# gooofy/zerovox

Hardware: AMD Instinct MI355X
Metric: audio samples/sec + RTF, 128-phoneme zero-shot synth @22.05kHz, 1/2/4/8 GPU (higher is better)
Workload: dtype f16+bf16

## Files before the change

### zerovox_amd/build.py

```python
import os
import subprocess
import sys

HERE = os.path.dirname(os.path.abspath(__file__))
CSRC = os.path.join(HERE, "csrc")
LIB = os.path.join(HERE, "libzvx.so")
KTEST_SRC = os.path.join(os.path.dirname(HERE), "tests", "native", "zvx_ktest.hip")
KTEST_LIB = os.path.join(HERE, "libzvx_ktest.so")
SOURCES = ["gemm.hip", "resstream.hip", "pairstream.hip", "narrowstage.hip", "attention.hip", "ops.hip", "spectral.hip", "zvx.hip"]
UNITS = [("gemm", "gemm.hip", ["-DZVX_GEMM_PART=1"]), ("gemm_resfuse", "gemm.hip", ["-DZVX_GEMM_PART=2"])] + \
        [(s_[:-4], s_, []) for s_ in SOURCES[1:]]
FLAGS = ["--offload-arch=gfx950", "-O3", "-std=c++17", "-fPIC", "-Wall", "-Wno-unused-function", "-Wno-inline-asm"]
EXTRA_FLAGS = {"gemm.hip": ["-fno-honor-nans"], "pairstream.hip": ["-fno-honor-nans"], "narrowstage.hip": ["-fno-honor-nans"], "resstream.hip": ["-fno-honor-nans"] + (["-DRS_PROFILE"] if os.environ.get("ZVX_RS_PROFILE_BUILD") else [])}


def _stale(target, deps):
    if not os.path.exists(target):
        return True
    t = os.path.getmtime(target)
    return any(os.path.getmtime(d) > t for d in deps)


def _parse_resources(text):
    import re
    res, cur = {}, None
    keys = {"TotalSGPRs": "sgprs", "VGPRs": "vgprs", "AGPRs": "agprs", "ScratchSize [bytes/lane]": "scratch", "Occupancy [waves/SIMD]": "occupancy",
            "SGPRs Spill": "sgpr_spill", "VGPRs Spill": "vgpr_spill", "LDS Size [bytes/block]": "lds"}
    for line in text.splitlines():
        m = re.search(r"remark:\s+Function Name: (\S+)", line)
        if m:
            cur = res.setdefault(m.group(1), {})
            continue
        m = re.search(r"remark:\s+([A-Za-z \[\]/]+): (\d+)", line)
        if m and cur is not None and m.group(1).strip() in keys:
            cur[keys[m.group(1).strip()]] = int(m.group(2))
    return res


def resources():
    import json
    out = {}
    for stem, _src, _defs in UNITS:
        f = os.path.join(CSRC, stem + ".resources.json")
        if os.path.exists(f):
            out.update(json.load(open(f)))
    return out


def build(force: bool = False, verbose: bool = True) -> str:
    hipcc = os.environ.get("HIPCC", "/opt/rocm/bin/hipcc")
    headers = [os.path.join(CSRC, "zvx_kernels.h"), os.path.join(CSRC, "mfma_util.h"), os.path.join(os.path.dirname(HERE), "include", "zvx.h")]
    def compile_one(unit):
        stem, src, defs = unit
        s = os.path.join(CSRC, src)
        o = os.path.join(CSRC, stem + ".o")
        rj = os.path.join(CSRC, stem + ".resources.json")
        if force or _stale(o, [s] + headers) or not os.path.exists(rj):
            cmd = [hipcc] + FLAGS + EXTRA_FLAGS.get(src, []) + defs + ["-Rpass-analysis=kernel-resource-usage", "-c", s, "-o", o]
            if verbose:
                print(" ".join(cmd), flush=True)
            p = subprocess.run(cmd, stderr=subprocess.PIPE, text=True)
            lines, keep, skip = p.stderr.splitlines(), [], 0
            for l in lines:
                if "[-Rpass-analysis=kernel-resource-usage]" in l:
                    skip = 2
                elif skip and (l.lstrip().startswith("|") or (l.strip()[:1].isdigit() and " | " in l)):
# ... 43 lines not shown
```

### zerovox_amd/csrc/gemm.hip

```cpp
#include "mfma_util.h"
#include "zvx_kernels.h"

#include <cstring>
#include <type_traits>

#ifndef ZVX_GEMM_PART
#define ZVX_GEMM_PART 0
#endif
#define ZVX_PART_MAIN (ZVX_GEMM_PART != 2)
#define ZVX_PART_RESFUSE (ZVX_GEMM_PART != 1)
#if ZVX_GEMM_PART == 2
extern thread_local bool zvx_gemm_dry_run;
#else
thread_local hipEvent_t zvx_gemm_ev_start = nullptr, zvx_gemm_ev_stop = nullptr;
thread_local bool zvx_gemm_dry_run = false;
#endif
#define g_dry_run zvx_gemm_dry_run

#define ZVX_LAUNCH(...) do { if (!g_dry_run) ZVX_DISPATCH(__VA_ARGS__); } while (0)

namespace zvx {


#define PITCH 80
// ... 774 lines not shown
    uint4 w[NT][KS];
    {
        const uint4* Wq = (const uint4*)a.Wp + ((long)wc * NT * 4) * 64 + lane;
#pragma unroll
        for (int t = 0; t < NT; t++)
#pragma unroll
            for (int kk = 0; kk < KS; kk++) w[t][kk] = Wq[(t * 4 + kk) * 64];
    }
    {
        const bool flat = MAXH > 64 && a.flat_win;
        const int in_rows = flat ? a.flat_rows : in_len;
#pragma unroll
        for (int h0 = 0; h0 < NIT; h0 += FCH) {
            uint4 sv[FCH];
#pragma unroll
            for (int i = 0; i < FCH; i++) {
                const int c = tid + (h0 + i) * 256;
                const int row = c / CPR, q = c % CPR;
                const int g = m0 - HL + row;
                sv[i] = make_uint4(0, 0, 0, 0);
                if (h0 + i < NIT && c < SR * CPR && g >= 0 && g < in_rows && (!flat || (g % a.flat_win) < in_len)) sv[i] = *(const uint4*)(Xp + (long)g * a.ldx + q * 8);
            }
#pragma unroll
            for (int i = 0; i < FCH; i++) {
                const int c = tid + (h0 + i) * 256;
                if (h0 + i < NIT && c < SR * CPR) *(uint4*)(slab + (c / CPR) * PITCH_ + (c % CPR) * 16) = sv[i];
            }
        }
    }
    __syncthreads();

    f32x16 acc[1][TM];
#pragma unroll
    for (int j = 0; j < TM; j++)
#pragma unroll
        for (int e = 0; e < 16; e++) acc[0][j][e] = 0.f;
    const int xrow0 = HL + wr * (BM / WM) + (lane & 31);
    const int koff = (lane >> 5) * 16;
#pragma unroll
    for (int t = 0; t < NT; t++) {
        const unsigned char* rowp = slab + (xrow0 + a.dv[t]) * PITCH_ + koff;
#pragma unroll
        for (int kk = 0; kk < KS; kk++)
#pragma unroll
            for (int j = 0; j < TM; j++) {
                const uint4 xf = *(const uint4*)(rowp + j * 32 * PITCH_ + kk * 32);
                acc[0][j] = mfma16<F16>(w[t][kk], xf, acc[0][j]);
            }
    }
    __syncthreads();
    epilogue_rows<TM, 1>(a, acc, b, m0 + wr * (BM / WM), wc * 32, out_len, lane, slab + wave * (32 * (32 * 4 + 16)));
}

typedef __attribute__((ext_vector_type(2))) unsigned u32x2_t;
__device__ __forceinline__ void store_block_mfma_layout(unsigned short* row_ptr , const uint2 (&pk)[4], int lane, bool ok) {
#pragma unroll
    for (int pr = 0; pr < 2; pr++) {
        const u32x2_t sx = __builtin_amdgcn_permlane32_swap(pk[2 * pr].x, pk[2 * pr + 1].x, false, false);
        const u32x2_t sy = __builtin_amdgcn_permlane32_swap(pk[2 * pr].y, pk[2 * pr + 1].y, false, false);
        if (ok) *(u32x4*)(row_ptr + 8 * (2 * pr + (lane >> 5))) = (u32x4){sx.x, sy.x, sx.y, sy.y};
    }
}

template <int C, int BM, int WM, int WN, int MAXH, int MODE, int WGPC, bool POOL = false>
__global__ __launch_bounds__(WM * WN * 64, WM * WN * WGPC / 4) void conv2d_persist_kernel(const GemmArgs a, const int ntm, const int ntiles) {
    constexpr int NTHR = WM * WN * 64;
    constexpr int NT = 9, TM = BM / WM / 32, KS = C / 16, PITCH_ = C * 2 + 16, CPR = C / 8, RSTEP = NTHR / CPR;
    constexpr int NIT = ((BM + MAXH) * CPR + NTHR - 1) / NTHR;
    constexpr bool EC_LDS = NTHR > 256;
    static_assert(WN * 32 == C && BM % (WM * 32) == 0, "wave layout");
    extern __shared__ __attribute__((aligned(16))) unsigned char slab[];

    const int tid = threadIdx.x, lane = tid & 63, wave = __builtin_amdgcn_readfirstlane(tid >> 6);
    const int wr = wave % WM, wc = wave / WM;
    const int G = gridDim.x, xcd = blockIdx.x & 7, slot = blockIdx.x >> 3;
    auto tile_of = [&](int r) {
        const int base = r * G, n = ntiles - base < G ? ntiles - base : G;
        if (n <= 0) return ntiles;
        const int per = (n + 7) >> 3, t = xcd * per + slot;
        return (slot < per && t < n) ? base + t : ntiles;
    };
    const int HL = a.halo_l, SR = BM + a.halo_l + a.halo_r, win = a.flat_win, in_rows = a.flat_rows;

    uint4 w[NT][KS];
    {
        const uint4* Wq = (const uint4*)a.Wp + ((long)wc * NT * 4) * 64 + lane;
#pragma unroll
        for (int t = 0; t < NT; t++)
#pragma unroll
            for (int kk = 0; kk < KS; kk++) w[t][kk] = Wq[(t * 4 + kk) * 64];
    }
    float* const ecl = (float*)(slab + ((SR * PITCH_ + 15) & ~15));
    float4 ec0[EC_LDS ? 1 : 4], ec1[(MODE == 1 && !EC_LDS) ? 4 : 1];
    if (EC_LDS) {
        if (tid < C) { ecl[tid] = MODE == 0 ? a.bias[tid] : a.post_scale[tid]; if (MODE == 1) ecl[C + tid] = a.post_shift[tid]; }
    } else {
#pragma unroll
        for (int g = 0; g < 4; g++) {
            const int ch = wc * 32 + 8 * g + 4 * (lane >> 5);
            if (MODE == 0) ec0[g] = *(const float4*)(a.bias + ch);
            else { ec0[g] = *(const float4*)(a.post_scale + ch); ec1[g] = *(const float4*)(a.post_shift + ch); }
        }
    }
    u32x4 sv[NIT];
    const int row_t = tid / CPR, q8 = (tid % CPR) * 8;
    auto request = [&](int t) __attribute__((always_inline)) {
        const int b = t / ntm, m0 = (t - b * ntm) * BM;
        const int in_len = a.in_len[b];
        const __amdgpu_buffer_rsrc_t rs = __builtin_amdgcn_make_buffer_rsrc((void*)((const unsigned short*)a.X + (long)b * a.x_bs), 0, in_rows * a.ldx * 2, 0x00020000);
        int g = m0 - HL + row_t;
        int col = (g + 2 * win) % win;
#pragma unroll
        for (int it = 0; it < NIT; it++) {
            const bool ok = tid + it * NTHR < SR * CPR && g >= 0 && g < in_rows && col < in_len;
            sv[it] = __builtin_amdgcn_raw_buffer_load_b128(rs, ok ? (g * a.ldx + q8) * 2 : (int)0x80000000, 0, 0);
// ... 761 lines not shown
        if (a.ntaps == 3) { ZVX_RFP_MODE(3) }
        if (a.ntaps == 7) { ZVX_RFP_MODE(7) }
        if constexpr (C <= 32) { if (a.ntaps == 11) { ZVX_RFP_MODE(11) } }
    }
#undef ZVX_RFP_MODE
#undef ZVX_RFP
    return false;
}

int launch_resfuse(GemmArgs a, hipStream_t stream) {
    if (a.dtype == DT_F32 || !a.Wp || !a.Wp2 || a.N != a.K || a.nheads != 1 || a.wout > 0) return -1;
    if (!(a.ntaps == 3 || a.ntaps == 7 || a.ntaps == 11)) return -1;
    int h1 = 0;
    for (int i = 0; i < a.ntaps; i++) { const int d = a.dv1[i] < 0 ? -a.dv1[i] : a.dv1[i]; if (d > h1) h1 = d; }
    if (h1 > 32) return -1;
    a.halo_l = a.halo_r = h1;
    a.fused = 1;
    if (a.N == 128 && a.no_pairstream != 1) {
        const int h2 = (a.ntaps - 1) / 2, dil = a.dv1[1] - a.dv1[0];
        bool ok = a.alpha == 1.f && a.bias_mode == 1 && !a.post_scale && (!a.out || a.out_dtype == a.dtype) && a.res_mode == 2 && a.res_dtype == a.dtype &&
                  a.res == a.X && a.r_bs == a.x_bs && a.ldr == a.ldx && (!a.accum || a.accum_dtype == a.dtype) && (a.act == ACT_NONE || a.act == ACT_LRELU) &&
                  (a.accum_mode || a.out_scale == 1.f) && a.in_len == a.out_len;
        for (int t = 0; t < a.ntaps; t++) ok = ok && a.dv[t] == t - h2 && a.dv1[t] == (t - h2) * dil;
        if (ok) {
            PairArgs p;
            memset(&p, 0, sizeof p);
            p.X = a.X; p.x_bs = a.x_bs; p.ldx = a.ldx; p.W1 = a.Wp2; p.W2 = a.Wp; p.b1 = a.bias1; p.b2 = a.bias;
            p.C = a.N; p.ntaps = a.ntaps; p.dil = dil;
            p.out = a.out; p.o_bs = a.o_bs; p.ldo = a.ldo;
            p.accum = a.accum; p.a_bs = a.a_bs; p.lda = a.lda; p.accum_mode = a.accum ? a.accum_mode : 0;
            p.slope1 = a.slope1; p.res_inv_slope = a.res_inv_slope; p.out_scale = a.out_scale; p.slope = a.act == ACT_LRELU ? a.slope : 1.f;
            p.f16 = a.dtype == DT_F16;
            p.len = a.out_len; p.M = a.M; p.nbatch = a.nbatch; p.force = a.no_pairstream == 2;
            if (launch_pairstream(p, stream, g_dry_run)) return 23;
        }
    }
    {
        if (a.N == 32 && launch_resfuse_persist_c<32>(a, stream)) return 16;
        if (a.N == 64 && a.ntaps != 11 && launch_resfuse_persist_c<64>(a, stream)) return 17;
        if (a.N == 64 && a.ntaps == 11 && launch_resfuse_persist_c<64, 1>(a, stream)) return 17;
    }
    return -1;
}
#endif
#if ZVX_PART_MAIN

struct Variant { const char* name; int dt, bm, bn; };
static const Variant kVariants[] = {
    {"gemm_bf16_128x128", DT_BF16, 128, 128}, {"gemm_bf16_256x64", DT_BF16, 256, 64},
    {"gemm_bf16_256x32", DT_BF16, 256, 32},   {"gemm_f32_128x128", DT_F32, 128, 128},
    {"gemm_f32_256x64", DT_F32, 256, 64},     {"gemm_f32_256x32", DT_F32, 256, 32},
    {"convslab_bf16_128x256", DT_BF16, 128, 256}, {"convslab_bf16_256x128", DT_BF16, 256, 128},
    {"convslab_bf16_256x64", DT_BF16, 256, 64},   {"convslab_bf16_256x32", DT_BF16, 256, 32},
    {"(unused)", DT_BF16, 0, 0}, {"resfuse_bf16_c8", DT_BF16, 256, 8}, {"resfuse_bf16_c16", DT_BF16, 256, 16}, {"resfuse_bf16_c128", DT_BF16, 64, 128},
    {"convreg_bf16_c32", DT_BF16, 512, 32},       {"convreg_bf16_c64", DT_BF16, 256, 64},
    {"resfuse_bf16_c32", DT_BF16, 256, 32},       {"resfuse_bf16_c64", DT_BF16, 128, 64},
    {"gemm_bf16_64x64", DT_BF16, 64, 64},         {"gemm_f32_64x64", DT_F32, 64, 64},
    {"resstream_bf16_c32", DT_BF16, 64, 32},      {"resstream_bf16_c64", DT_BF16, 32, 64},
    {"convslab_bf16_128x128", DT_BF16, 128, 128},
    {"pairstream_bf16_c128", DT_BF16, 128, 128},
    {"narrowstage_c16", DT_BF16, 256, 16}, {"narrowstage_c8", DT_BF16, 512, 8},
    {"conv2d_persist_c32", DT_BF16, 384, 32}, {"conv2d_persist_c64", DT_BF16, 256, 64},
    {"conv2d_s2_c32", DT_BF16, 256, 64}, {"conv2d_s2_c64", DT_BF16, 128, 128},
    {"rb2fuse_bf16_c32", DT_BF16, 256, 32}, {"rb2fuse_bf16_c64", DT_BF16, 256, 64},
};
const char* gemm_variant_name(int id) { return kVariants[id].name; }
int gemm_num_variants() { return (int)(sizeof(kVariants) / sizeof(kVariants[0])); }


template <int BM, int BN, int WM, int WN, int MINW, int R, int EPI = -1>
static void launch_slab_variant(const GemmArgs& a, dim3 grid, size_t lds, hipStream_t stream) {
    const bool fullk = a.K % SLAB_KC == 0 && a.K2 == 0;
    if constexpr (R == 0 || EPI == -1 || EPI == ZVX_EPI(0, 0, 1) || EPI == ZVX_EPI_FLIP) {
        if (a.dtype == DT_F16) {
            if (fullk) ZVX_LAUNCH((convslab_kernel<BM, BN, WM, WN, true, MINW, R, EPI, 64, true>), grid, dim3(256), lds, stream, a);
            else if constexpr (EPI != ZVX_EPI_FLIP) ZVX_LAUNCH((convslab_kernel<BM, BN, WM, WN, false, MINW, R, EPI, 64, true>), grid, dim3(256), lds, stream, a);
            return;
        }
    }
    if constexpr (EPI < 0 || !(EPI & 16)) {
        if (fullk) ZVX_LAUNCH((convslab_kernel<BM, BN, WM, WN, true, MINW, R, EPI>), grid, dim3(256), lds, stream, a);
        else if constexpr (EPI != ZVX_EPI_FLIP) ZVX_LAUNCH((convslab_kernel<BM, BN, WM, WN, false, MINW, R, EPI>), grid, dim3(256), lds, stream, a);
    }
}

int gemm_epi_mode_of(const GemmArgs& a) {
    if (a.alpha == 1.f && !a.post_scale && a.out && a.out_dtype != a.dtype && a.dtype != DT_F32 && a.out_dtype != DT_F32 && !a.out_split3 && a.bias_mode == 1 && a.bias &&
        (a.act == ACT_NONE || a.act == ACT_LRELU) && !a.res_mode && !(a.accum && a.accum_mode) && a.out_scale == 1.f && a.K % SLAB_KC == 0 && !a.K2) return ZVX_EPI_FLIP;
    if (a.alpha != 1.f || a.post_scale || (a.out && a.out_dtype != a.dtype) || a.dtype == DT_F32 || a.out_split3 || a.bias_mode == 2) return -1;
    const int am = a.accum ? a.accum_mode : 0;
    if (a.dtype == DT_F16 && a.out && !am && a.act == ACT_NONE && a.res_mode <= 1 && (!a.res_mode || a.res_dtype == DT_F16) && (a.res_mode || a.out_scale != 1.f) &&
        (a.bias_mode == 0 || a.bias)) return ZVX_EPI_DEC(a.res_mode ? 1 : 0);
    if (a.bias_mode != 1 || !a.bias) return -1;
    if (a.act != ACT_NONE && a.act != ACT_LRELU) return -1;
    if (a.res_mode && (a.res_mode != 2 || a.res_dtype != a.dtype)) return -1;
    if (am && a.accum_dtype != a.dtype) return -1;
    if (!am && a.out_scale != 1.f) return -1;
    if (!a.out && !(am & 2)) return -1;
    const int e = ZVX_EPI(a.res_mode ? 1 : 0, am, a.out ? 1 : 0);
    switch (e) {
        case ZVX_EPI(0, 0, 1): case ZVX_EPI(1, 0, 1): case ZVX_EPI(1, 2, 0): case ZVX_EPI(1, 3, 0): case ZVX_EPI(1, 1, 1): return e;
    }
    return -1;
}

static int launch_convslab(GemmArgs a, hipStream_t stream) {
    const bool bflat_hint = a.bflat != 0;
// ... 247 lines not shown
```

### zerovox_amd/csrc/mfma_util.h

```cpp
#pragma once
#include <hip/hip_runtime.h>

namespace zvx {

typedef __attribute__((ext_vector_type(8))) __bf16 bf16x8;
typedef __attribute__((ext_vector_type(16))) float f32x16;
typedef __attribute__((ext_vector_type(4))) float f32x4;
typedef __attribute__((ext_vector_type(4))) unsigned int u32x4;
typedef __attribute__((ext_vector_type(4))) int i32x4;
typedef float f32x2 __attribute__((ext_vector_type(2)));

__device__ __forceinline__ unsigned pack_bf16x2(float lo, float hi) {
    typedef __attribute__((ext_vector_type(2))) __bf16 bf16x2_t;
    bf16x2_t v = {(__bf16)lo, (__bf16)hi};
    return __builtin_bit_cast(unsigned, v);
}
__device__ __forceinline__ f32x2 unpack_bf16x2(unsigned u) { return (f32x2){__uint_as_float(u << 16), __uint_as_float(u & 0xffff0000u)}; }
__device__ __forceinline__ f32x2 lrelu2(f32x2 v, float slope) { const f32x2 m = v * slope; return (f32x2){fmaxf(v.x, m.x), fmaxf(v.y, m.y)}; }
__device__ __forceinline__ f32x2 inv_lrelu2(f32x2 y, float inv_slope) { const f32x2 m = y * inv_slope; return (f32x2){fminf(y.x, m.x), fminf(y.y, m.y)}; }

typedef __attribute__((ext_vector_type(8))) _Float16 f16x8;
typedef _Float16 f16x2_t __attribute__((ext_vector_type(2)));
__device__ __forceinline__ void f16_saturate_mode() { asm volatile("s_setreg_imm32_b32 hwreg(HW_REG_MODE, 23, 1), 1"); }
__device__ __forceinline__ unsigned pack_f16x2_raw(float lo, float hi) { const f16x2_t v = {(_Float16)lo, (_Float16)hi}; return __builtin_bit_cast(unsigned, v); }
__device__ __forceinline__ unsigned pack_f16x2_sat(float lo, float hi) { return pack_f16x2_raw(__builtin_amdgcn_fmed3f(lo, -65504.f, 65504.f), __builtin_amdgcn_fmed3f(hi, -65504.f, 65504.f)); }
__device__ __forceinline__ f32x2 unpack_f16x2(unsigned u) { const f16x2_t v = __builtin_bit_cast(f16x2_t, u); return (f32x2){(float)v.x, (float)v.y}; }
template <bool H> __device__ __forceinline__ unsigned pack16(float lo, float hi) { if constexpr (H) return pack_f16x2_raw(lo, hi); else return pack_bf16x2(lo, hi); }
template <bool H> __device__ __forceinline__ f32x2 unpack16(unsigned u) { if constexpr (H) return unpack_f16x2(u); else return unpack_bf16x2(u); }
template <bool H> __device__ __forceinline__ f32x16 mfma16(const uint4& a, const uint4& b, const f32x16& c) {
    if constexpr (H) return __builtin_amdgcn_mfma_f32_32x32x16_f16(__builtin_bit_cast(f16x8, a), __builtin_bit_cast(f16x8, b), c, 0, 0, 0);
    else return __builtin_amdgcn_mfma_f32_32x32x16_bf16(__builtin_bit_cast(bf16x8, a), __builtin_bit_cast(bf16x8, b), c, 0, 0, 0);
}
template <bool H> __device__ __forceinline__ f32x16 mfma16(const u32x4& a, const uint4& b, const f32x16& c) { return mfma16<H>(__builtin_bit_cast(uint4, a), b, c); }

}
```

### zerovox_amd/csrc/zvx.hip

```cpp
#include "../../include/zvx.h"
#include "zvx_kernels.h"

#include <dlfcn.h>
#include <math.h>
#include <cmath>
#include <rccl/rccl.h>
#include <stdarg.h>
#include <stdio.h>
#include <string.h>

#include <algorithm>
#include <map>
#include <sstream>
#include <stdexcept>
#include <string>
#include <vector>

using namespace zvx;

namespace {

struct ZvxError : std::runtime_error {
    int code;
    ZvxError(int c, const std::string& m) : std::runtime_error(m), code(c) {}
// ... 47 lines not shown
    hipEvent_t ev_aux[2] = {nullptr, nullptr};
    int va_overlap_maxb = 1 << 20;
    ncclComm_t comm = nullptr;
    int rank = 0, world = 1;
    hipEvent_t ev_compute = nullptr;
    std::map<const void*, hipEvent_t> gather_fence;
    std::string err;
    std::map<std::string, std::string> cfg;
    std::map<std::string, Tensor> tensors;
    std::vector<float> host_blob;
    std::map<std::string, DevBuf> bufs;
    std::map<const void*, const void*> packed;
    std::map<const void*, const void*> pair_packed;
    int dt = DT_BF16;
    int H = 0, emb_dim = 0, punct_dim = 0, n_phone_rows = 0, n_punct_rows = 0, max_txt_len = 0, max_mel_len = 0;
    int enc_layers = 0, enc_heads = 0, ffn_dim = 0, ffn_k0 = 0, ffn_k1 = 0, vp_dim = 0, vp_k = 0, n_bins = 0;
    int dec_layers = 0, dec_heads = 0, dec_scln = 0, n_mels = 0, hop = 0, res_dim = 0, dec_kind = 0, rn_asp = 1;
    std::vector<int> rn_layers, rn_filters, voc_rates, voc_ksizes, voc_rb_k;
    std::vector<std::vector<int>> voc_rb_d;
    int voc_resblock = 1, voc_c0 = 0;
    int B = 0, Tmax = 0, Lmax = 0;
    std::vector<int> T_host, mel_len_host;
    std::vector<int> in_stage;
    bool have_features = false, have_mel = false;
    int profile = 0;
    int profile_only = -1;
    int rs_prof = 0;
    int enc_split = 0;
    const void* fft_xs_ready = nullptr;
    int norm_fuse_maxb = 1 << 20;
    int dec_sc_fuse = 1;
    int dec_flat = 1;
    int voc_f16_stages = -1;
    int voc_h16_ok = -1;
    int voc_f16 = 1;
    int dec_f16 = 1;
    int use_attn_f32 = 1;
    int use_flash = 1;
    int use_resstream = 1;
    int rs_seg_min = 0;
    int spk_s2_fuse = 1;
    int spk_pool_fuse = 1;
    int slab_small = 2, slab_flat = 1;
    int poison_pads = 0;
    int sat_check = 0;
    unsigned long long* sat_count_dev() { return (unsigned long long*)buf("sat.count", 64); }
    void sat_scan(const void* x, int dt, long bs, int ld, int B, int rows_max, const int* rows, int C) {
        if (sat_check && x && dt == DT_F16) launch_count_sat16(x, bs, ld, B, rows_max, rows, C, sat_count_dev(), stream);
    }
    int use_rb2fuse = 1;
    int use_stagefuse = 1;
    struct NsWeights { void* W = nullptr; float* bias = nullptr; int woff[18] = {0}; };
    std::map<std::string, NsWeights> ns_weights;
    int use_pairstream = 1;
    int shape_log = 0;
    int max_frames = 1 << 18;
    int out_rate = 0;
    struct RsBank { int L = 0, M = 0, half = 0, T = 0, pitch = 0; const float* dev = nullptr; };
    std::map<std::pair<int, int>, RsBank> rs_banks;
    std::map<int, const double*> lim_wins;
    std::map<int, LoudCoef> loud_coefs;
    struct DnTables { int n_fft = 0, log2n = 0, win_length = 0; const float* twid = nullptr; const float* win = nullptr; const double* win2 = nullptr; double den_min = 0; };
    DnTables dn_tab;
    void* join_host = nullptr;
    size_t join_host_cap = 0;
    void* join_pinned(size_t bytes) {
        if (bytes > join_host_cap) {
            if (join_host) { HIPCHK(hipStreamSynchronize(stream)); HIPCHK(hipHostFree(join_host)); join_host = nullptr; join_host_cap = 0; }
            const size_t cap = bytes + bytes / 8 + 256;
            HIPCHK(hipHostMalloc(&join_host, cap, hipHostMallocDefault));
            join_host_cap = cap;
        }
        return join_host;
    }
    hipEvent_t stage_ev[ZVX_T_COUNT][2];
    bool stage_used[ZVX_T_COUNT];
    float stage_ms[ZVX_T_COUNT];
    std::vector<GemmEvent> pending;
    std::vector<zvx_kernel_stat> stats;
    std::string tag = "other";
    std::map<std::string, zvx_kernel_stat> tagstats;
    std::map<std::string, zvx_kernel_stat> namedstats;
    std::vector<hipEvent_t> event_pool;

    int cfg_int(const char* k) const {
        auto it = cfg.find(k);
        if (it == cfg.end()) fail(ZVX_E_MANIFEST, "manifest: missing cfg '%s'", k);
        return atoi(it->second.c_str());
    }
    std::vector<int> cfg_list(const char* k) const {
        auto it = cfg.find(k);
        if (it == cfg.end()) fail(ZVX_E_MANIFEST, "manifest: missing cfg '%s'", k);
        std::vector<int> v; std::stringstream ss(it->second); std::string tok;
        while (std::getline(ss, tok, ',')) if (!tok.empty()) v.push_back(atoi(tok.c_str()));
        return v;
    }
    const Tensor& t(const std::string& name) const {
        auto it = tensors.find(name);
        if (it == tensors.end()) fail(ZVX_E_MANIFEST, "weights: tensor '%s' missing", name.c_str());
        return it->second;
    }
    bool has(const std::string& name) const { return tensors.count(name) != 0; }
    const float* pf(const std::string& name) const { return (const float*)t(name).dev; }

    void drain_for_free() {
        HIPCHK(hipStreamSynchronize(stream));
// ... 1010 lines not shown
struct VocStage {
    int i, Cin, Cout, rows_in, rows;
    const int* len_in; const int* len;
    int dt_in, dt;
    float next_slope;
};

struct RbConv { std::string name; const Tensor* w = nullptr; const void* packed = nullptr; const float* bias = nullptr; };
struct RbWeights { std::string name; std::vector<RbConv> c1, c2; };
RbWeights voc_rb_weights(zvx_ctx* c, const VocCall& v, const VocStage& s, int j) {
    RbWeights w;
    w.name = "voc.rb" + std::to_string(s.i * v.nk + j);
    auto conv = [&](const char* which, int t) {
        RbConv r;
        r.name = w.name + which + std::to_string(t);
        r.w = &voc_weight(c, r.name + "_w", s.dt);
        auto it = c->packed.find(r.w->dev);
        if (it != c->packed.end()) r.packed = it->second;
        r.bias = c->pf(r.name + "_b");
        return r;
    };
    for (int t = 0; t < (int)c->voc_rb_d[j].size(); t++) {
        if (c->voc_resblock == 1) { w.c1.push_back(conv(".c1_", t)); w.c2.push_back(conv(".c2_", t)); }
        else w.c1.push_back(conv(".c_", t));
    }
    return w;
}

struct StageClose { int accum_mode; bool writes_out; };
StageClose stage_close(int j, int nk) {
    if (nk == 1) return {0, true};
    return {j == 0 ? 2 : (j < nk - 1 ? 3 : 1), j == nk - 1};
}
template <typename Args>
void close_stage(Args& a, const StageClose& cl, const VocCall& v, const VocStage& s) {
    a.accum = cl.accum_mode ? v.XS : nullptr; a.accum_mode = cl.accum_mode; a.a_bs = (long)s.rows * s.Cout; a.lda = s.Cout;
    if (cl.writes_out) { a.out = v.A; a.out_scale = 1.0f / v.nk; a.slope = s.next_slope; }
    else a.out = nullptr;
    if constexpr (std::is_same<Args, GemmArgs>::value) { a.accum_dtype = s.dt; if (cl.writes_out) a.act = ACT_LRELU; }
}

void voc_conv_pre(zvx_ctx* c, const VocCall& v, const void* vin, int dt) {
    const int nm = c->n_mels, Pmax = v.Pmax;
    const int* P_d = v.lens_d + v.B;
    GemmArgs a = gemm_base(dt);
    a.X = vin; a.x_bs = (long)Pmax * nm; a.ldx = nm; a.W = voc_weight(c, "voc.pre_w", dt).dev; a.ldw = nm; a.w_ts = (long)c->voc_c0 * nm;
    a.M = Pmax; a.N = c->voc_c0; a.K = nm; a.nbatch = v.B; a.in_len = P_d; a.out_len = P_d;
    set_taps_1d(a, c->t("voc.pre_w").dim(0), 1);
    a.bias = c->pf("voc.pre_b"); a.bias_mode = 1; a.act = ACT_LRELU; a.slope = 0.1f;
    a.out = v.A; a.o_bs = (long)Pmax * c->voc_c0; a.ldo = c->voc_c0;
    c->gemm(a);
}

void voc_upsample(zvx_ctx* c, const VocCall& v, const VocStage& s) {
    const int u = c->voc_rates[s.i], ku = c->voc_ksizes[s.i], B = v.B, Cin = s.Cin, Cout = s.Cout, rows_in = s.rows_in, dt_in = s.dt_in;
    const std::string up = "voc.up" + std::to_string(s.i);
    GemmArgs a = gemm_base(dt_in);
    a.out_dtype = s.dt;
    a.X = v.A; a.x_bs = (long)rows_in * Cin; a.ldx = Cin; a.ldw = Cin;
    a.M = rows_in; a.K = Cin; a.nbatch = B; a.in_len = s.len_in; a.out_len = s.len_in;
    a.bias_mode = 1; a.act = ACT_LRELU; a.slope = 0.1f;
    a.o_bs = (long)rows_in * u * Cout; a.ldo = u * Cout;
    if (dt_in != DT_F32 && c->has(up + "_wlo")) {
        const int hc = (u / 2) * Cout;
        a.N = hc; a.ntaps = 2; a.w_ts = (long)hc * Cin; a.flops = 2.0 * B * (double)rows_in * Cin * Cout * ku / 2;
        a.W = voc_weight(c, up + "_wlo", dt_in).dev; a.dv[0] = -1; a.dv[1] = 0;
        a.bias = c->pf(up + "_b"); a.out = v.X0;
        c->gemm(a);
        a.Wp = nullptr;
        a.W = voc_weight(c, up + "_whi", dt_in).dev; a.dv[0] = 0; a.dv[1] = 1;
        a.bias = c->pf(up + "_b") + hc; a.out = (char*)v.X0 + (size_t)hc * c->es();
        c->gemm(a);
    } else {
        a.W = voc_weight(c, up + "_w", dt_in).dev; a.w_ts = (long)u * Cout * Cin; a.N = u * Cout;
        a.ntaps = 3; a.dv[0] = -1; a.dv[1] = 0; a.dv[2] = 1;
        a.bias = c->pf(up + "_b"); a.out = v.X0;
        a.flops = 2.0 * B * (double)rows_in * Cin * Cout * ku;
        c->gemm(a);
    }
}

const zvx_ctx::NsWeights& voc_narrow_weights(zvx_ctx* c, const VocCall& v, const VocStage& s) {
    const int Cout = s.Cout, nk = v.nk;
    const std::string key = "voc.ns." + std::to_string(s.i) + (s.dt == DT_F16 ? ".h16" : "");
    auto it = c->ns_weights.find(key);
    if (it != c->ns_weights.end()) return it->second;
    zvx_ctx::NsWeights nw;
    int nfrag = 0;
    for (int j = 0; j < nk; j++) for (int q = 0; q < 6; q++) { nw.woff[6 * j + q] = nfrag; nfrag += narrowstage_steps(Cout, c->voc_rb_k[j]); }
    nw.W = c->buf(key + ".w", (size_t)nfrag * 1024);
    nw.bias = c->fbuf(key + ".b", (size_t)6 * nk * Cout);
    for (int j = 0; j < nk; j++) {
        const RbWeights w = voc_rb_weights(c, v, s, j);
        for (int t = 0; t < 3; t++)
            for (int q = 0; q < 2; q++) {
                const RbConv& cv = q ? w.c2[t] : w.c1[t];
                if (cv.w->dims.size() != 3 || cv.w->dim(0) != c->voc_rb_k[j] || cv.w->dim(1) != Cout || cv.w->dim(2) != Cout) fail(ZVX_E_MANIFEST, "weights: '%s' has an unexpected shape", cv.name.c_str());
                const int ci = 6 * j + 2 * t + q;
                launch_pack_narrow(cv.w->dev, c->voc_rb_k[j], Cout, (char*)nw.W + (size_t)nw.woff[ci] * 1024, c->stream);
                HIPCHK(hipMemcpyAsync(nw.bias + (size_t)ci * Cout, cv.bias, (size_t)Cout * 4, hipMemcpyDeviceToDevice, c->stream));
            }
    }
    return c->ns_weights.emplace(key, nw).first->second;
}

bool voc_narrow_stage(zvx_ctx* c, const VocCall& v, const VocStage& s) {
    const int Cout = s.Cout, nk = v.nk, rows = s.rows;
    if (!c->use_stagefuse || c->sat_check || c->voc_resblock != 1 || s.dt == DT_F32 || (Cout != 16 && Cout != 8) || nk < 1 || nk > 3) return false;
    for (int j = 0; j < nk; j++) if (c->voc_rb_d[j].size() != 3) return false;
// ... 1230 lines not shown
    (void)hipSetDevice(c->device);
    if (c->front_stream) (void)hipStreamSynchronize(c->front_stream);
    if (c->stream) (void)hipStreamSynchronize(c->stream);
    zvx_comm_destroy(c);
    for (int i = 0; i < 2; i++) { if (c->arena[i].p) (void)hipHostFree(c->arena[i].p); if (c->arena[i].ev) (void)hipEventDestroy(c->arena[i].ev); }
    if (c->copy_stream && !c->copy_is_comm) { (void)hipStreamSynchronize(c->copy_stream); (void)hipStreamDestroy(c->copy_stream); }
    for (auto& hs : c->host_slot) { if (hs.p) (void)hipHostFree(hs.p); if (hs.ready) (void)hipEventDestroy(hs.ready); if (hs.done) (void)hipEventDestroy(hs.done); }
    if (c->join_host) (void)hipHostFree(c->join_host);
    for (int i = 0; i < 2; i++) if (c->voc_aux[i]) { (void)hipStreamSynchronize(c->voc_aux[i]); (void)hipStreamDestroy(c->voc_aux[i]); }
    for (int i = 0; i < 3; i++) if (c->voc_ev[i]) (void)hipEventDestroy(c->voc_ev[i]);
    if (c->aux_stream) { (void)hipStreamSynchronize(c->aux_stream); (void)hipStreamDestroy(c->aux_stream); (void)hipEventDestroy(c->ev_aux[0]); (void)hipEventDestroy(c->ev_aux[1]); }
    if (c->front_stream) {
        (void)hipStreamSynchronize(c->front_stream); (void)hipStreamDestroy(c->front_stream);
        (void)hipEventDestroy(c->ev_front_done); (void)hipEventDestroy(c->ev_mel_free); (void)hipEventDestroy(c->ev_main_join);
    }
    for (auto& kv : c->bufs) if (kv.second.base) (void)hipFree(kv.second.base);
    for (auto e : c->event_pool) (void)hipEventDestroy(e);
    if (c->stream) {
        for (int s = 0; s < ZVX_T_COUNT; s++) { (void)hipEventDestroy(c->stage_ev[s][0]); (void)hipEventDestroy(c->stage_ev[s][1]); }
        (void)hipStreamDestroy(c->stream);
    }
    delete c;
}

const char* zvx_last_error(const zvx_ctx* c) { return c ? c->err.c_str() : g_create_error.c_str(); }

namespace {

struct Switch { const char* key; int zvx_ctx::*v; bool (*ok)(int64_t); };
bool flag(int64_t v) { return v == 0 || v == 1; }
bool count(int64_t v) { return v >= 0 && v <= INT32_MAX; }
const Switch kSwitches[] = {
    {"profile", &zvx_ctx::profile, [](int64_t v) { return v >= 0 && v <= 2; }},
    {"profile_only", &zvx_ctx::profile_only, [](int64_t v) { return v >= -1 && v < gemm_num_variants(); }},
    {"shape_log", &zvx_ctx::shape_log, flag},
    {"rs_prof", &zvx_ctx::rs_prof, flag},
    {"f16_sat_check", &zvx_ctx::sat_check, flag},
    {"poison_pads", &zvx_ctx::poison_pads, flag},
    {"max_frames", &zvx_ctx::max_frames, [](int64_t v) { return v >= 1 && v <= (1 << 24); }},
    {"enc_split", &zvx_ctx::enc_split, [](int64_t v) { return v >= 0 && v <= 2; }},
    {"attn_f32", &zvx_ctx::use_attn_f32, flag},
    {"flash", &zvx_ctx::use_flash, flag},
    {"front_overlap", &zvx_ctx::front_overlap, [](int64_t v) { return v >= 0 && v <= 2; }},
    {"va_overlap_maxb", &zvx_ctx::va_overlap_maxb, count},
    {"dec_f16", &zvx_ctx::dec_f16, flag},
    {"dec_flat", &zvx_ctx::dec_flat, flag},
    {"dec_sc_fuse", &zvx_ctx::dec_sc_fuse, flag},
    {"norm_fuse_maxb", &zvx_ctx::norm_fuse_maxb, count},
    {"voc_f16", &zvx_ctx::voc_f16, flag},
    {"voc_f16_stages", &zvx_ctx::voc_f16_stages, [](int64_t v) { return v >= -1 && v <= INT32_MAX; }},
    {"voc_overlap_maxb", &zvx_ctx::voc_overlap_maxb, count},
    {"voc_overlap_frames", &zvx_ctx::voc_overlap_frames, count},
    {"stagefuse", &zvx_ctx::use_stagefuse, flag},
    {"rb2fuse", &zvx_ctx::use_rb2fuse, flag},
    {"resstream", &zvx_ctx::use_resstream, flag},
    {"rs_seg_min", &zvx_ctx::rs_seg_min, [](int64_t v) { return v >= -1 && v <= INT32_MAX; }},
    {"pairstream", &zvx_ctx::use_pairstream, [](int64_t v) { return v == -1 || v == 0 || v == 1 || v == 3; }},
    {"slab_small", &zvx_ctx::slab_small, [](int64_t v) { return (v & ~32) >= 0 && (v & ~32) <= 2; }},
    {"slab_flat", &zvx_ctx::slab_flat, flag},
    {"spk_pool_fuse", &zvx_ctx::spk_pool_fuse, flag},
    {"spk_s2_fuse", &zvx_ctx::spk_s2_fuse, flag},
    {"out_rate", &zvx_ctx::out_rate, count},
};
const Switch* find_switch(const char* key) {
    for (const Switch& s : kSwitches) if (!strcmp(s.key, key)) return &s;
    return nullptr;
}

}

int64_t zvx_get_int(const zvx_ctx* c, const char* key) {
    if (!c || !key) return -1;
    if (const Switch* s = find_switch(key)) return c->*s->v;
    const std::string k(key);
    if (k == "precision") return c->dt == DT_F32 ? 1 : 0;
    if (k == "hidden") return c->H;
    if (k == "n_mels") return c->n_mels;
    if (k == "hop") return c->hop;
    if (k == "device") return c->device;
    if (k == "dec_kind") return c->dec_kind;
    if (k == "Lmax") return c->Lmax;
    if (k == "f16_sat_events") {
        zvx_ctx* m = const_cast<zvx_ctx*>(c);
        unsigned long long n = 0;
        if (hipSetDevice(m->device) != hipSuccess) return -1;
        try { unsigned long long* d = m->sat_count_dev(); m->sync(); if (hipMemcpy(&n, d, sizeof n, hipMemcpyDeviceToHost) != hipSuccess) return -1; } catch (...) { return -1; }
        return (int64_t)n;
    }
    if (k == "host_slot") return c->host_last;
    if (k.rfind("variant_id:", 0) == 0) { for (int i = 0; i < gemm_num_variants(); i++) if (k.substr(11) == gemm_variant_name(i)) return i; return -1; }
    auto it = c->cfg.find(k);
    if (it != c->cfg.end()) return atoll(it->second.c_str());
    return -1;
}

zvx_status zvx_set_int(zvx_ctx* c, const char* key, int64_t value) {
    return guarded(c, [&] {
        if (!key) fail(ZVX_E_INVALID, "key is NULL");
        const Switch* s = find_switch(key);
        if (!s) fail(ZVX_E_INVALID, "unknown option '%s'", key);
        if (!s->ok(value)) fail(ZVX_E_INVALID, "option '%s' does not take the value %lld", key, (long long)value);
        const std::string k(key);
        if (k == "out_rate" && value) {
            int L = 1, M = 1;
            rs_pair(model_rate(c), (int)value, &L, &M);
            if ((int)value != model_rate(c)) rs_bank(c, L, M);
// ... 489 lines not shown
```

### zerovox_amd/csrc/zvx_kernels.h

```cpp
#pragma once
#include <hip/hip_runtime.h>
#include <hip/hip_ext.h>
#include <stdint.h>
#include <atomic>
#include <mutex>
#include <set>
#include <utility>

extern thread_local hipEvent_t zvx_gemm_ev_start, zvx_gemm_ev_stop;
#define ZVX_DISPATCH(kernel, grid, block, lds, stream, ...) \
    do { if (zvx_gemm_ev_start) hipExtLaunchKernelGGL(kernel, grid, block, lds, stream, zvx_gemm_ev_start, zvx_gemm_ev_stop, 0, __VA_ARGS__); \
         else hipLaunchKernelGGL(kernel, grid, block, lds, stream, __VA_ARGS__); } while (0)

namespace zvx {

inline void profile_events(hipEvent_t start, hipEvent_t stop) { zvx_gemm_ev_start = start; zvx_gemm_ev_stop = stop; }

typedef unsigned short bf16_t;

enum DType { DT_F32 = 0, DT_BF16 = 1, DT_F16 = 2 };
static inline size_t dtype_size(int dt) { return dt == DT_F32 ? 4 : 2; }
inline int num_cus() {
    static const int n = [] { int dev = 0, v = 0; if (hipGetDevice(&dev) != hipSuccess || hipDeviceGetAttribute(&v, hipDeviceAttributeMultiprocessorCount, dev) != hipSuccess || v <= 0) v = 256; return v; }();
    return n;
// ... 64 lines not shown
const char* gemm_variant_name(int id);
int gemm_num_variants();

struct StreamArgs {
    const void* X; long x_bs; int ldx;
    const void* W1[3]; const void* W2[3];
    const float* b1[3]; const float* b2[3];
    int dil[3];
    int C, ntaps, npair;
    void* out; long o_bs; int ldo;
    void* accum; long a_bs; int lda; int accum_mode;
    float slope1, res_inv_slope, out_scale, slope;
    const int* len; int M, nbatch;
    int S, nseg;
    int dX0, dT, dX[3];
    double flops;
    long long* prof;
    int seg_min;
    int f16;
};
int launch_resstream(StreamArgs a, hipStream_t stream, bool dry_run);

struct PairArgs {
    const void* X; long x_bs; int ldx;
    const void* W1; const void* W2;
    const float* b1; const float* b2;
    int C, ntaps, dil;
    void* out; long o_bs; int ldo;
    void* accum; long a_bs; int lda; int accum_mode;
    float slope1, res_inv_slope, out_scale, slope;
    const int* len; int M, nbatch;
    int force;
    int f16;
    int S, nseg, DX, DT, G0;
    long long* prof;
};
bool launch_pairstream(PairArgs a, hipStream_t stream, bool dry_run);

struct StageArgs {
    const void* X; long x_bs; int ldx;
    const void* W;
    int woff[18];
    const float* bias;
    int C, nk, ks[3], dil[3][3];
    void* out; long o_bs; int ldo;
    float slope1, res_inv_slope, slope;
    const int* len; int M, nbatch;
    int f16;
};
bool launch_narrowstage(const StageArgs& a, hipStream_t stream, bool dry_run);
int narrowstage_steps(int C, int k);
void launch_pack_narrow(const void* w16 , int k, int C, void* out, hipStream_t s);

struct FlashArgs {
    const void* qk; long qk_bs; int ldq; int k_off;
    const void* vt; long vt_bs; int ldv;
    void* out; long o_bs; int ldo;
    const int* len; int L, D, nheads, nbatch;
    float scale;
    int f16;
    long long* prof;
};
bool launch_flash_attention(const FlashArgs& a, hipStream_t stream, bool dry_run);
struct AttnF32Args {
    const float* qkv; long bs; int ld; int q_off, k_off, v_off;
    float* out; long o_bs; int ldo;
    unsigned short* planes; int planes_C;
    int planes_f16;
    const int* len; int L, D, nheads, nbatch;
    float scale;
};
bool launch_attention_f32(const AttnF32Args& a, hipStream_t stream, bool dry_run);

void launch_instnorm_fused(const void* x, int x_dt, int ldx, void* y, int y_dt, int ldy, int B, int Lmax, const int* L, int C, float eps,
                           float* mean, float* rstd, const float* gamma, const float* beta, long g_bs, int one_plus, int act, float slope, hipStream_t s);
void launch_transpose16(const void* in, int ld_in, void* out, int ld_out, int B, int rows, int C, hipStream_t s, const int* len = nullptr);
void launch_f32_to_bf16(const float* in, bf16_t* out, size_t n, hipStream_t s);
void launch_zero_tail_cols(void* x, int es, long ld, long bs, int B, int rows, int cols, const int* len, hipStream_t s);
void launch_cast(const void* in, int in_dt, void* out, int out_dt, size_t n, hipStream_t s);

void launch_split3(const float* x, int ldx, void* out, int B, int rows_max, const int* rows, int C, hipStream_t s, int f16 = 0);
void launch_split3_weights(const float* w, void* out, long nrows, int K, hipStream_t s, int f16 = 0, float scale = 1.f);
void launch_absmax(const float* x, size_t n, float* out , hipStream_t s);

void launch_embed(const int* phoneme, const int* puncts, const float* emb, int emb_dim, const float* pemb,
                  int pemb_dim, const float* pe, float* out, int B, int Tmax, const int* T, hipStream_t s);

void launch_layernorm(const void* x, int x_dt, int ldx, void* y, int y_dt, int ldy, int B, int rows_max,
                      const int* rows, int C, int mode, float eps, const float* gamma, const float* beta,
                      const float* bg, long bg_bs, const float* post_add, hipStream_t s, void* split_planes = nullptr, int planes_f16 = 0);

void launch_softmax_rows(const float* scores, int lds, void* P, int p_dt, int ldp, int nbatch, int nheads,
                         int Lmax, const int* len, hipStream_t s);

void launch_rowdot(const float* x, int ldx, const float* w, float bias, float* out, int B, int Tmax,
                   const int* T, int C, hipStream_t s);

void launch_bucket_embed_add(const float* pred, const float* table, int nbins, float* x, int ldx, int C,
                             int* idx_out, int B, int Tmax, const int* T, hipStream_t s);

void launch_durations(const int* forced, const float* logd, int* dur, int* cum, int* mel_len, int B, int Tmax,
                      const int* T, hipStream_t s);

void launch_bucket_embed_add_ctl(const float* pred, const float* shift, const float* range, const float* target, const float* table,
                                 int nbins, float* x, int ldx, int C, int* idx_out, int B, int Tmax, const int* T, hipStream_t s);
void launch_durations_q16(const int* forced, const float* logd, const int* q, int* dur, int* cum, int* mel_len, int B, int Tmax,
// ... 125 lines not shown
```

Before: 344.0 million.

## Add persistent MFMA kernel for stride-2 vocoder transposed-conv upsample stages

Adds a dedicated persistent kernel for the vocoder's rate-2, kernel-4 transposed-convolution upsample stages (128->64 and 64->32 channels). It keeps pre-packed weights in registers, stages input rows in LDS with prefetch of the next tile, and fuses bias plus leaky-ReLU into the epilogue. This replaces the generic GEMM path for those stages and is enabled by default. Weights are packed once and cached per stage. The kernel only handles specific channel shapes and needs extra LDS.

Result: no change. 346.1 million, median of 6 (+0.6%).

```diff
diff --git a/zerovox_amd/build.py b/zerovox_amd/build.py
--- a/zerovox_amd/build.py
+++ b/zerovox_amd/build.py
@@ -7,11 +7,11 @@
 LIB = os.path.join(HERE, "libzvx.so")
 KTEST_SRC = os.path.join(os.path.dirname(HERE), "tests", "native", "zvx_ktest.hip")
 KTEST_LIB = os.path.join(HERE, "libzvx_ktest.so")
-SOURCES = ["gemm.hip", "resstream.hip", "pairstream.hip", "narrowstage.hip", "attention.hip", "ops.hip", "spectral.hip", "zvx.hip"]
+SOURCES = ["gemm.hip", "convtr2.hip", "resstream.hip", "pairstream.hip", "narrowstage.hip", "attention.hip", "ops.hip", "spectral.hip", "zvx.hip"]
 UNITS = [("gemm", "gemm.hip", ["-DZVX_GEMM_PART=1"]), ("gemm_resfuse", "gemm.hip", ["-DZVX_GEMM_PART=2"])] + \
         [(s_[:-4], s_, []) for s_ in SOURCES[1:]]
 FLAGS = ["--offload-arch=gfx950", "-O3", "-std=c++17", "-fPIC", "-Wall", "-Wno-unused-function", "-Wno-inline-asm"]
-EXTRA_FLAGS = {"gemm.hip": ["-fno-honor-nans"], "pairstream.hip": ["-fno-honor-nans"], "narrowstage.hip": ["-fno-honor-nans"], "resstream.hip": ["-fno-honor-nans"] + (["-DRS_PROFILE"] if os.environ.get("ZVX_RS_PROFILE_BUILD") else [])}
+EXTRA_FLAGS = {"gemm.hip": ["-fno-honor-nans"], "convtr2.hip": ["-fno-honor-nans"], "pairstream.hip": ["-fno-honor-nans"], "narrowstage.hip": ["-fno-honor-nans"], "resstream.hip": ["-fno-honor-nans"] + (["-DRS_PROFILE"] if os.environ.get("ZVX_RS_PROFILE_BUILD") else [])}
 
 
 def _stale(target, deps):
diff --git a/zerovox_amd/csrc/convtr2.hip b/zerovox_amd/csrc/convtr2.hip
--- /dev/null
+++ b/zerovox_amd/csrc/convtr2.hip
@@ -0,0 +1,175 @@
+#include "mfma_util.h"
+#include "zvx_kernels.h"
+
+namespace zvx {
+
+__global__ void k_pack_convtr2(const unsigned short* w, int Cin, int Cout, unsigned short* out, int total_frag_lanes) {
+    const int idx = blockIdx.x * blockDim.x + threadIdx.x;
+    if (idx >= total_frag_lanes) return;
+    const int KS = Cin / 16, N = 2 * Cout;
+    const int lane = idx & 63;
+    int t = idx >> 6;
+    const int kk = t % KS; t /= KS;
+    const int ts = t & 1, ct = t >> 1;
+    const int n = ct * 32 + (lane & 31), tap = n / Cout + ts;
+    *(uint4*)(out + (long)idx * 8) = *(const uint4*)(w + ((long)tap * N + n) * Cin + kk * 16 + 8 * (lane >> 5));
+}
+
+size_t convtr2_packed_bytes(int Cin, int Cout) { return (size_t)(2 * Cout / 32) * 2 * (Cin / 16) * 1024; }
+
+void launch_pack_convtr2(const void* w16, int Cin, int Cout, void* out, hipStream_t s) {
+    const int total = (2 * Cout / 32) * 2 * (Cin / 16) * 64;
+    hipLaunchKernelGGL(k_pack_convtr2, dim3((total + 255) / 256), dim3(256), 0, s, (const unsigned short*)w16, Cin, Cout, (unsigned short*)out, total);
+}
+
+#define CT2_BM 256
+
+template <int CIN, int COUT, bool IN_F16, bool OUT_F16>
+__global__ __launch_bounds__(256, 2) void convtr2_persist_kernel(const ConvTr2Args a, const int ntm, const int ntiles) {
+    constexpr int N = 2 * COUT, WN = N / 32, WM = 4 / WN, NTHR = 256;
+    constexpr int BM = CT2_BM, TM = BM / WM / 32, KS = CIN / 16, PITCH_ = CIN * 2 + 16, CPR = CIN / 8, RSTEP = NTHR / CPR;
+    constexpr int SR = BM + 2, NCH = SR * CPR, NIT = (NCH + NTHR - 1) / NTHR;
+    static_assert(WM * WN == 4 && COUT % 32 == 0 && CIN % 64 == 0 && TM % 2 == 0, "wave layout");
+    extern __shared__ __attribute__((aligned(16))) unsigned char slab[];
+
+    const int tid = threadIdx.x, lane = tid & 63, wave = __builtin_amdgcn_readfirstlane(tid >> 6);
+    const int wr = wave % WM, wc = wave / WM;
+    const int ph = (wc * 32) / COUT;
+    const int G = gridDim.x, xcd = blockIdx.x & 7, slot = blockIdx.x >> 3;
+    auto tile_of = [&](int r) {
+        const int base = r * G, n = ntiles - base < G ? ntiles - base : G;
+        if (n <= 0) return ntiles;
+        const int per = (n + 7) >> 3, t = xcd * per + slot;
+        return (slot < per && t < n) ? base + t : ntiles;
+    };
+    auto next_tile = [&](int& r) {
+        for (;;) {
+            const int t = tile_of(r);
+            if (t >= ntiles) return ntiles;
+            const int b = t / ntm, m0 = (t - b * ntm) * BM;
+            if (m0 < a.len[b]) return t;
+            r++;
+        }
+    };
+
+    uint4 w[2][KS];
+    {
+        const uint4* Wq = (const uint4*)a.Wp + ((long)wc * 2 * KS) * 64 + lane;
+#pragma unroll
+        for (int ts = 0; ts < 2; ts++)
+#pragma unroll
+            for (int kk = 0; kk < KS; kk++) w[ts][kk] = Wq[(ts * KS + kk) * 64];
+    }
+    float4 bb[4];
+#pragma unroll
+    for (int g = 0; g < 4; g++) bb[g] = *(const float4*)(a.bias + wc * 32 + 8 * g + 4 * (lane >> 5));
+    const float slope = a.slope;
+
+    u32x4 sv[NIT];
+    const int row_t = tid / CPR, q8 = (tid % CPR) * 8;
+    auto request = [&](int t) __attribute__((always_inline)) {
+        const int b = t / ntm, m0 = (t - b * ntm) * BM;
+        const int len = a.len[b];
+        const __amdgpu_buffer_rsrc_t rs = __builtin_amdgcn_make_buffer_rsrc((void*)((const unsigned short*)a.X + (long)b * a.x_bs), 0, a.M * a.ldx * 2, 0x00020000);
+        int g = m0 - 1 + row_t;
+#pragma unroll
+        for (int it = 0; it < NIT; it++) {
+            const bool ok = tid + it * NTHR < NCH && g >= 0 && g < len;
+            sv[it] = __builtin_amdgcn_raw_buffer_load_b128(rs, ok ? (g * a.ldx + q8) * 2 : (int)0x80000000, 0, 0);
+            g += RSTEP;
+        }
+    };
+    int r = 0, t = next_tile(r);
+    if (t < ntiles) request(t);
+    const int xrow0 = ph + wr * (BM / WM) + (lane & 31);
+    const int koff = (lane >> 5) * 16;
+    bool first = true;
+    while (t < ntiles) {
+        const int b = t / ntm, m0 = (t - b * ntm) * BM;
+        const int len = a.len[b];
+        if (!first) __syncthreads();
+        first = false;
+        int ts_ = tid;
+        asm volatile("" : "+v"(ts_));
+#pragma unroll
+        for (int it = 0; it < NIT; it++) {
+            const int c = ts_ + it * NTHR;
+            if (c < NCH) *(u32x4*)(slab + (c / CPR) * PITCH_ + (c % CPR) * 16) = sv[it];
+        }
+        __syncthreads();
+        r++;
+        const int tn = next_tile(r);
+        if (tn < ntiles) request(tn);
+
+        unsigned short* const ob = (unsigned short*)a.out + (long)b * a.o_bs + wc * 32;
+        const int row0 = m0 + wr * (BM / WM) + (lane & 31);
+#pragma unroll 1
+        for (int j0 = 0; j0 < TM; j0 += 2) {
+            if (m0 + wr * (BM / WM) + j0 * 32 >= len) break;
+            f32x16 acc[2];
+#pragma unroll
+            for (int jj = 0; jj < 2; jj++)
+#pragma unroll
+                for (int e = 0; e < 16; e++) acc[jj][e] = 0.f;
+            const unsigned char* rowp = slab + (xrow0 + j0 * 32) * PITCH_ + koff;
+#pragma unroll
+            for (int kc = 0; kc < CIN / 64; kc++)
+#pragma unroll
+                for (int ts = 0; ts < 2; ts++)
+#pragma unroll
+                    for (int k16 = 0; k16 < 4; k16++) {
+                        const int kk = kc * 4 + k16;
+#pragma unroll
+                        for (int jj = 0; jj < 2; jj++) {
+                            const uint4 xf = *(const uint4*)(rowp + (jj * 32 + ts) * PITCH_ + kk * 32);
+                            acc[jj] = mfma16<IN_F16>(w[ts][kk], xf, acc[jj]);
+                        }
+                    }
+#pragma unroll
+            for (int jj = 0; jj < 2; jj++) {
+                const int row = row0 + (j0 + jj) * 32;
+                uint2 pk[4];
+#pragma unroll
+                for (int g = 0; g < 4; g++) {
+                    const f32x2 v01 = lrelu2((f32x2){acc[jj][4 * g], acc[jj][4 * g + 1]} + (f32x2){bb[g].x, bb[g].y}, slope);
+                    const f32x2 v23 = lrelu2((f32x2){acc[jj][4 * g + 2], acc[jj][4 * g + 3]} + (f32x2){bb[g].z, bb[g].w}, slope);
+                    if (OUT_F16) pk[g] = make_uint2(pack_f16x2_sat(v01.x, v01.y), pack_f16x2_sat(v23.x, v23.y));
+                    else pk[g] = make_uint2(pack_bf16x2(v01.x, v01.y), pack_bf16x2(v23.x, v23.y));
+                }
+                store_block_mfma_layout(ob + (long)row * a.ldo, pk, lane, row < len);
+            }
+        }
+        t = tn;
+    }
+}
+
+template <int CIN, int COUT>
+static bool launch_convtr2_c(const ConvTr2Args& a, hipStream_t stream, bool dry_run) {
+    const size_t lds = (size_t)(CT2_BM + 2) * (CIN * 2 + 16);
+    const int ntm = (a.M + CT2_BM - 1) / CT2_BM;
+    if ((long)ntm * a.nbatch >= (1L << 30)) return false;
+    const int ntiles = ntm * a.nbatch;
+    int G = (2 * persistent_cus()) & ~7;
+    if (G < 8) G = 8;
+    if (ntiles < G) G = (ntiles + 7) & ~7;
+    if (a.max_wgs > 0 && a.max_wgs < G) G = a.max_wgs < 8 ? a.max_wgs : (a.max_wgs & ~7);
+#define ZVX_CT2(I, O) do { \
+        if (lds > 64 * 1024 && !lds_opt_in((const void*)convtr2_persist_kernel<CIN, COUT, I, O>)) return false; \
+        if (!dry_run) ZVX_DISPATCH((convtr2_persist_kernel<CIN, COUT, I, O>), dim3(G), dim3(256), lds, stream, a, ntm, ntiles); } while (0)
+    if (a.in_f16) { if (a.out_f16) ZVX_CT2(true, true); else ZVX_CT2(true, false); }
+    else { if (a.out_f16) ZVX_CT2(false, true); else ZVX_CT2(false, false); }
+#undef ZVX_CT2
+    return true;
+}
+
+bool launch_convtr2(const ConvTr2Args& a, hipStream_t stream, bool dry_run) {
+    if (!a.X || !a.Wp || !a.bias || !a.out || !a.len || a.M <= 0 || a.nbatch <= 0) return false;
+    if (a.ldx != a.Cin || a.ldo != 2 * a.Cout || a.x_bs % 8 || a.o_bs % 8 || ((uintptr_t)a.X & 15) || ((uintptr_t)a.out & 15) || ((uintptr_t)a.Wp & 15) || ((uintptr_t)a.bias & 15)) return false;
+    if ((long)a.M * a.ldx * 2 >= 0x7fffffffL) return false;
+    if (!(a.slope >= 0.f && a.slope <= 1.f)) return false;
+    if (a.Cin == 128 && a.Cout == 64) return launch_convtr2_c<128, 64>(a, stream, dry_run);
+    if (a.Cin == 64 && a.Cout == 32) return launch_convtr2_c<64, 32>(a, stream, dry_run);
+    return false;
+}
+
+}
diff --git a/zerovox_amd/csrc/gemm.hip b/zerovox_amd/csrc/gemm.hip
--- a/zerovox_amd/csrc/gemm.hip
+++ b/zerovox_amd/csrc/gemm.hip
@@ -850,15 +850,6 @@
     epilogue_rows<TM, 1>(a, acc, b, m0 + wr * (BM / WM), wc * 32, out_len, lane, slab + wave * (32 * (32 * 4 + 16)));
 }
 
-typedef __attribute__((ext_vector_type(2))) unsigned u32x2_t;
-__device__ __forceinline__ void store_block_mfma_layout(unsigned short* row_ptr , const uint2 (&pk)[4], int lane, bool ok) {
-#pragma unroll
-    for (int pr = 0; pr < 2; pr++) {
-        const u32x2_t sx = __builtin_amdgcn_permlane32_swap(pk[2 * pr].x, pk[2 * pr + 1].x, false, false);
-        const u32x2_t sy = __builtin_amdgcn_permlane32_swap(pk[2 * pr].y, pk[2 * pr + 1].y, false, false);
-        if (ok) *(u32x4*)(row_ptr + 8 * (2 * pr + (lane >> 5))) = (u32x4){sx.x, sy.x, sx.y, sy.y};
-    }
-}
 
 template <int C, int BM, int WM, int WN, int MAXH, int MODE, int WGPC, bool POOL = false>
 __global__ __launch_bounds__(WM * WN * 64, WM * WN * WGPC / 4) void conv2d_persist_kernel(const GemmArgs a, const int ntm, const int ntiles) {
@@ -1726,7 +1717,8 @@
     {"gemm_f32_256x64", DT_F32, 256, 64},     {"gemm_f32_256x32", DT_F32, 256, 32},
     {"convslab_bf16_128x256", DT_BF16, 128, 256}, {"convslab_bf16_256x128", DT_BF16, 256, 128},
     {"convslab_bf16_256x64", DT_BF16, 256, 64},   {"convslab_bf16_256x32", DT_BF16, 256, 32},
-    {"(unused)", DT_BF16, 0, 0}, {"resfuse_bf16_c8", DT_BF16, 256, 8}, {"resfuse_bf16_c16", DT_BF16, 256, 16}, {"resfuse_bf16_c128", DT_BF16, 64, 128},
+    {"convtr2_bf16_c128", DT_BF16, 256, 128}, {"convtr2_bf16_c64", DT_BF16, 256, 64},
+     {"resfuse_bf16_c16", DT_BF16, 256, 16}, {"resfuse_bf16_c128", DT_BF16, 64, 128},
     {"convreg_bf16_c32", DT_BF16, 512, 32},       {"convreg_bf16_c64", DT_BF16, 256, 64},
     {"resfuse_bf16_c32", DT_BF16, 256, 32},       {"resfuse_bf16_c64", DT_BF16, 128, 64},
     {"gemm_bf16_64x64", DT_BF16, 64, 64},         {"gemm_f32_64x64", DT_F32, 64, 64},
diff --git a/zerovox_amd/csrc/mfma_util.h b/zerovox_amd/csrc/mfma_util.h
--- a/zerovox_amd/csrc/mfma_util.h
+++ b/zerovox_amd/csrc/mfma_util.h
@@ -33,4 +33,14 @@
 }
 template <bool H> __device__ __forceinline__ f32x16 mfma16(const u32x4& a, const uint4& b, const f32x16& c) { return mfma16<H>(__builtin_bit_cast(uint4, a), b, c); }
 
+typedef __attribute__((ext_vector_type(2))) unsigned u32x2_t;
+__device__ __forceinline__ void store_block_mfma_layout(unsigned short* row_ptr , const uint2 (&pk)[4], int lane, bool ok) {
+#pragma unroll
+    for (int pr = 0; pr < 2; pr++) {
+        const u32x2_t sx = __builtin_amdgcn_permlane32_swap(pk[2 * pr].x, pk[2 * pr + 1].x, false, false);
+        const u32x2_t sy = __builtin_amdgcn_permlane32_swap(pk[2 * pr].y, pk[2 * pr + 1].y, false, false);
+        if (ok) *(u32x4*)(row_ptr + 8 * (2 * pr + (lane >> 5))) = (u32x4){sx.x, sy.x, sx.y, sy.y};
+    }
 }
+
+}
diff --git a/zerovox_amd/csrc/zvx.hip b/zerovox_amd/csrc/zvx.hip
--- a/zerovox_amd/csrc/zvx.hip
+++ b/zerovox_amd/csrc/zvx.hip
@@ -123,6 +123,9 @@
     int use_stagefuse = 1;
     struct NsWeights { void* W = nullptr; float* bias = nullptr; int woff[18] = {0}; };
     std::map<std::string, NsWeights> ns_weights;
+    int use_up_persist = 1;
+    int up_persist_wgs = 0;
+    std::map<std::string, const void*> ct2_weights;
     int use_pairstream = 1;
     int shape_log = 0;
     int max_frames = 1 << 18;
@@ -1239,9 +1242,48 @@
     c->gemm(a);
 }
 
+const void* voc_convtr2_weights(zvx_ctx* c, const VocStage& s) {
+    const std::string key = "voc.ct2." + std::to_string(s.i) + (s.dt_in == DT_F16 ? ".h16" : "");
+    auto it = c->ct2_weights.find(key);
+    if (it != c->ct2_weights.end()) return it->second;
+    void* pk = c->buf(key, convtr2_packed_bytes(s.Cin, s.Cout));
+    launch_pack_convtr2(voc_weight(c, "voc.up" + std::to_string(s.i) + "_w", s.dt_in).dev, s.Cin, s.Cout, pk, c->stream);
+    return c->ct2_weights.emplace(key, pk).first->second;
+}
+
+bool voc_upsample_persist(zvx_ctx* c, const VocCall& v, const VocStage& s) {
+    const int u = c->voc_rates[s.i], ku = c->voc_ksizes[s.i], Cin = s.Cin, Cout = s.Cout;
+    if (!c->use_up_persist || c->sat_check || s.dt_in == DT_F32 || s.dt == DT_F32 || u != 2 || ku != 4) return false;
+    if (!((Cin == 128 && Cout == 64) || (Cin == 64 && Cout == 32))) return false;
+    const std::string up = "voc.up" + std::to_string(s.i);
+    const Tensor& w = voc_weight(c, up + "_w", s.dt_in);
+    if (w.dims.size() != 3 || w.dim(0) != 3 || w.dim(1) != 2 * Cout || w.dim(2) != Cin) return false;
+    ConvTr2Args ca;
+    memset(&ca, 0, sizeof ca);
+    ca.X = v.A; ca.x_bs = (long)s.rows_in * Cin; ca.ldx = Cin;
+    ca.bias = c->pf(up + "_b");
+    ca.out = v.X0; ca.o_bs = (long)s.rows_in * 2 * Cout; ca.ldo = 2 * Cout;
+    ca.Cin = Cin; ca.Cout = Cout; ca.in_f16 = s.dt_in == DT_F16; ca.out_f16 = s.dt == DT_F16;
+    ca.slope = 0.1f; ca.len = s.len_in; ca.M = s.rows_in; ca.nbatch = v.B; ca.max_wgs = c->up_persist_wgs;
+    ca.Wp = w.dev;
+    if (!launch_convtr2(ca, c->stream, true)) return false;
+    ca.Wp = voc_convtr2_weights(c, s);
+    const int vid = Cin == 128 ? 10 : 11;
+    c->profiled([&] { return vid; }, [&] {
+        if (!launch_convtr2(ca, c->stream, false)) fail(ZVX_E_INVALID, "launch_convtr2 rejected a stage its dry run accepted (Cin=%d)", Cin);
+        return vid;
+    }, [&](GemmEvent& ev) {
+        const double rws = (double)s.rows_in * v.B;
+        ev.flops = 2.0 * rws * Cin * Cout * ku; ev.rows = (long)rws; ev.N = 2 * Cout; ev.K = Cin; ev.taps = 2;
+        ev.bytes = rws * (Cin + 2.0 * Cout) * 2.0 + (double)convtr2_packed_bytes(Cin, Cout);
+    });
+    return true;
+}
+
 void voc_upsample(zvx_ctx* c, const VocCall& v, const VocStage& s) {
     const int u = c->voc_rates[s.i], ku = c->voc_ksizes[s.i], B = v.B, Cin = s.Cin, Cout = s.Cout, rows_in = s.rows_in, dt_in = s.dt_in;
     const std::string up = "voc.up" + std::to_string(s.i);
+    if (voc_upsample_persist(c, v, s)) return;
     GemmArgs a = gemm_base(dt_in);
     a.out_dtype = s.dt;
     a.X = v.A; a.x_bs = (long)rows_in * Cin; a.ldx = Cin; a.ldw = Cin;
@@ -2578,6 +2620,8 @@
     {"voc_overlap_maxb", &zvx_ctx::voc_overlap_maxb, count},
     {"voc_overlap_frames", &zvx_ctx::voc_overlap_frames, count},
     {"stagefuse", &zvx_ctx::use_stagefuse, flag},
+    {"up_persist", &zvx_ctx::use_up_persist, flag},
+    {"up_persist_wgs", &zvx_ctx::up_persist_wgs, count},
     {"rb2fuse", &zvx_ctx::use_rb2fuse, flag},
     {"resstream", &zvx_ctx::use_resstream, flag},
     {"rs_seg_min", &zvx_ctx::rs_seg_min, [](int64_t v) { return v >= -1 && v <= INT32_MAX; }},
diff --git a/zerovox_amd/csrc/zvx_kernels.h b/zerovox_amd/csrc/zvx_kernels.h
--- a/zerovox_amd/csrc/zvx_kernels.h
+++ b/zerovox_amd/csrc/zvx_kernels.h
@@ -140,6 +140,21 @@
 int narrowstage_steps(int C, int k);
 void launch_pack_narrow(const void* w16 , int k, int C, void* out, hipStream_t s);
 
+struct ConvTr2Args {
+    const void* X; long x_bs; int ldx;
+    const void* Wp;
+    const float* bias;
+    void* out; long o_bs; int ldo;
+    int Cin, Cout;
+    int in_f16, out_f16;
+    float slope;
+    const int* len; int M, nbatch;
+    int max_wgs;
+};
+bool launch_convtr2(const ConvTr2Args& a, hipStream_t stream, bool dry_run);
+size_t convtr2_packed_bytes(int Cin, int Cout);
+void launch_pack_convtr2(const void* w16, int Cin, int Cout, void* out, hipStream_t s);
+
 struct FlashArgs {
     const void* qk; long qk_bs; int ldq; int k_off;
     const void* vt; long vt_bs; int ldv;
```
